# SimeonZhang/detectron2_tensorflow

Measured on AMD Instinct MI355X. Metric: img/sec whole-node Mask R-CNN R50-FPN @1333x800, higher is better.
Workload: dtype f32

## Files before the change

detectron2_tensorflow_amd/csrc/roi_align.hip:

```cpp
#include "common.h"
#include "internal.h"

#include <climits>

namespace d2mi {
namespace {

struct RoiArgs {
  const float* feat[D2MI_MAX_LEVELS];
  float* gfeat[D2MI_MAX_LEVELS];
  int N[D2MI_MAX_LEVELS], H[D2MI_MAX_LEVELS], W[D2MI_MAX_LEVELS];
  float scale[D2MI_MAX_LEVELS];
  int L, C;
  const float* boxes;
  const int32_t* box_ind;
  int R;
  int out_h, out_w, sr, box_mode, pad_border, assign;
  int min_level, max_level, canon_size, canon_level;
  int32_t* level_out;
  float* out;
  const float* gout;
  int32_t* err;
  int bpb;
  int xcd_remap;
// ... 77 lines not shown

__device__ __forceinline__ Tap make_tap(float in, int img_p, int img, bool pad) {
  Tap t;
  t.valid = in >= 0.f && in <= (float)(img_p - 1);
  const float fl = floorf(in);
  const int lo = (int)fl;
  const int hi = (int)ceilf(in);
  t.lerp = in - (float)lo;
  if (pad) {
    t.r0 = min(max(lo - 1, 0), img - 1);
    t.r1 = min(max(hi - 1, 0), img - 1);
  } else {
    t.r0 = min(max(lo, 0), img - 1);
    t.r1 = min(max(hi, 0), img - 1);
  }
  return t;
}

__device__ __forceinline__ float4 lerp4(float4 a, float4 b, float t) {
  return make_float4(a.x + (b.x - a.x) * t, a.y + (b.y - a.y) * t, a.z + (b.z - a.z) * t,
                     a.w + (b.w - a.w) * t);
}

constexpr int kMaxBinsPerBlock = 64, kMinBinsPerBlock = 16, kFwdMinBlocks = 2048;

template <bool VEC4, int U = 4, bool NT = false>
__global__ __launch_bounds__(256) void roi_align_fwd_kernel(RoiArgs a) {
  int r = blockIdx.x;
  if (a.xcd_remap) {
    const int nwg = gridDim.x, q = nwg / 8, r8 = nwg % 8, xcd = r % 8;
    r = (xcd < r8 ? xcd * (q + 1) : r8 * (q + 1) + (xcd - r8) * q) + r / 8;
  }
  const int wave = threadIdx.x >> 6;
  const int lane = threadIdx.x & 63;
  const RoiGeom g = roi_geom(a, r);
  if (threadIdx.x == 0 && blockIdx.y == 0) {
    if (a.level_out) a.level_out[r] = g.lvl;
    if (!g.ok) atomicOr(a.err, kErrBoxInd);
  }
  const int nbins = a.out_h * a.out_w;
  const int S = a.sr > 0 ? a.sr : 1;
  const float inv = a.sr > 0 ? (float)(a.sr * a.sr) : 1.f;
  const float* base = a.feat[g.lvl] + (size_t)(g.ok ? g.n : 0) * g.H * g.W * a.C;
  const int C = a.C;
  const bool pad = a.pad_border != 0;
  const int b_end = min(nbins, (int)(blockIdx.y + 1) * a.bpb);
  if (VEC4 && S == 1 && C == 256) {
    const float4* p = reinterpret_cast<const float4*>(base);
    for (int bb = blockIdx.y * a.bpb + wave; bb < b_end; bb += 4 * U) {
      float4 c00[U], c01[U], c10[U], c11[U];
      float ly[U], lx[U];
      bool ok[U];
#pragma unroll
      for (int u = 0; u < U; ++u) {
        const int bin = min(bb + 4 * u, b_end - 1);
        const int oy = bin / a.out_w, ox = bin - oy * a.out_w;
        const Tap ty = make_tap(in_coord(g.y1, g.y2, g.hs, oy, g.ch, g.Hp), g.Hp, g.H, pad);
        const Tap tx = make_tap(in_coord(g.x1, g.x2, g.ws, ox, g.cw, g.Wp), g.Wp, g.W, pad);
        ok[u] = g.ok && ty.valid && tx.valid;
        ly[u] = ty.lerp;
        lx[u] = tx.lerp;
        c00[u] = p[((size_t)ty.r0 * g.W + tx.r0) * 64 + lane];
        c01[u] = p[((size_t)ty.r0 * g.W + tx.r1) * 64 + lane];
        c10[u] = p[((size_t)ty.r1 * g.W + tx.r0) * 64 + lane];
        c11[u] = p[((size_t)ty.r1 * g.W + tx.r1) * 64 + lane];
      }
#pragma unroll
      for (int u = 0; u < U; ++u) {
        const int bin = bb + 4 * u;
        if (bin >= b_end) break;
        const float4 top = lerp4(c00[u], c01[u], lx[u]);
        const float4 bot = lerp4(c10[u], c11[u], lx[u]);
        const float4 v = ok[u] ? lerp4(top, bot, ly[u]) : make_float4(0.f, 0.f, 0.f, 0.f);
        float4* dst = reinterpret_cast<float4*>(a.out + ((size_t)r * nbins + bin) * C) + lane;
        if (NT) {
          typedef float f4v __attribute__((ext_vector_type(4)));
          __builtin_nontemporal_store(f4v{v.x, v.y, v.z, v.w}, reinterpret_cast<f4v*>(dst));
        } else
          *dst = v;
      }
    }
    return;
  }
  for (int bin = blockIdx.y * a.bpb + wave; bin < b_end; bin += 4) {
    const int oy = bin / a.out_w, ox = bin - oy * a.out_w;
    float* dst = a.out + ((size_t)r * nbins + bin) * C;
    if (VEC4) {
      for (int c4 = lane; c4 * 4 < C; c4 += 64) {
        float4 acc = make_float4(0.f, 0.f, 0.f, 0.f);
        if (g.ok) {
          for (int sy = 0; sy < S; ++sy) {
            const Tap ty = make_tap(in_coord(g.y1, g.y2, g.hs, oy * S + sy, g.ch, g.Hp), g.Hp,
                                    g.H, pad);
            for (int sx = 0; sx < S; ++sx) {
              const Tap tx = make_tap(in_coord(g.x1, g.x2, g.ws, ox * S + sx, g.cw, g.Wp),
                                      g.Wp, g.W, pad);
              float4 v = make_float4(0.f, 0.f, 0.f, 0.f);
              if (ty.valid && tx.valid) {
                const float4* p = reinterpret_cast<const float4*>(base);
                const float4 tl = p[((size_t)ty.r0 * g.W + tx.r0) * (C / 4) + c4];
                const float4 tr = p[((size_t)ty.r0 * g.W + tx.r1) * (C / 4) + c4];
                const float4 bl = p[((size_t)ty.r1 * g.W + tx.r0) * (C / 4) + c4];
                const float4 br = p[((size_t)ty.r1 * g.W + tx.r1) * (C / 4) + c4];
                const float4 top = lerp4(tl, tr, tx.lerp);
                const float4 bot = lerp4(bl, br, tx.lerp);
                v = lerp4(top, bot, ty.lerp);
              }
              if (S == 1) {
                acc = v;
              } else {
                acc.x += v.x; acc.y += v.y; acc.z += v.z; acc.w += v.w;
              }
            }
          }
          if (S > 1) { acc.x /= inv; acc.y /= inv; acc.z /= inv; acc.w /= inv; }
        }
        reinterpret_cast<float4*>(dst)[c4] = acc;
      }
    } else {
      for (int c = lane; c < C; c += 64) {
        float acc = 0.f;
        if (g.ok) {
          for (int sy = 0; sy < S; ++sy) {
            const Tap ty = make_tap(in_coord(g.y1, g.y2, g.hs, oy * S + sy, g.ch, g.Hp), g.Hp,
                                    g.H, pad);
            for (int sx = 0; sx < S; ++sx) {
              const Tap tx = make_tap(in_coord(g.x1, g.x2, g.ws, ox * S + sx, g.cw, g.Wp),
                                      g.Wp, g.W, pad);
              float v = 0.f;
              if (ty.valid && tx.valid) {
                const float tl = base[((size_t)ty.r0 * g.W + tx.r0) * C + c];
                const float tr = base[((size_t)ty.r0 * g.W + tx.r1) * C + c];
                const float bl = base[((size_t)ty.r1 * g.W + tx.r0) * C + c];
                const float br = base[((size_t)ty.r1 * g.W + tx.r1) * C + c];
                const float top = tl + (tr - tl) * tx.lerp;
                const float bot = bl + (br - bl) * tx.lerp;
                v = top + (bot - top) * ty.lerp;
              }
              acc = (S == 1) ? v : acc + v;
            }
          }
          if (S > 1) acc = acc / inv;
        }
        dst[c] = acc;
      }
    }
  }
}

constexpr int kSeg = 64;
constexpr int kBatch = 2;
constexpr int kLongTask = 1024;
constexpr int kLongTile = 4096;

struct PixMap {
  long long base[D2MI_MAX_LEVELS + 1];
  int32_t tbase[D2MI_MAX_LEVELS + 1];
  int L;
};

struct Contrib {
  int32_t row;
  float yl, xl;
  int32_t set;
};

struct RunRec {
  int32_t slot;
  int32_t row;
  float yl, xl;
};

struct BwdCounters {
  int32_t touched, segs, tasks, cursor;
  int32_t touched_lv[D2MI_MAX_LEVELS];
  int32_t touched_hv[D2MI_MAX_LEVELS];
  int32_t lsdone;
};

struct TouchedRange {
  int32_t pre[D2MI_MAX_LEVELS + 1];
  int32_t hv[D2MI_MAX_LEVELS];
  int lo, hi;
  __device__ __forceinline__ void init(const PixMap& pm, const BwdCounters* ctr, int lv_lo,
                                       int lv_hi) {
    lo = lv_lo;
    hi = lv_hi;
    pre[0] = 0;
#pragma unroll
    for (int j = 0; j < D2MI_MAX_LEVELS; ++j) {
      const bool in = j <= hi - lo;
      hv[j] = in ? ctr->touched_hv[lo + j] : 0;
      pre[j + 1] = pre[j] + (in ? ctr->touched_lv[lo + j] + hv[j] : 0);
    }
  }
  __device__ __forceinline__ int total() const {
    int v = 0;
#pragma unroll
    for (int j = 0; j <= D2MI_MAX_LEVELS; ++j) v = j == hi - lo + 1 ? pre[j] : v;
    return v;
  }
  __device__ __forceinline__ long long at(const PixMap& pm, const int32_t* touched, int t,
                                          int& l) const {
    return touched[index(pm, t, l)];
  }
  __device__ __forceinline__ int index(const PixMap& pm, int t, int& l) const {
    int k = 0, base = 0, h = hv[0];
#pragma unroll
    for (int j = 1; j < D2MI_MAX_LEVELS; ++j)
      if (j <= hi - lo && t >= pre[j]) {
        k = j;
        base = pre[j];
        h = hv[j];
      }
    l = lo + k;
    const int kk = t - base;
    return kk < h ? pm.tbase[l + 1] - 1 - kk : pm.tbase[l] + (kk - h);
  }
};

constexpr int kMaxClear = D2MI_MAX_LEVELS + 2;
struct ClearList {
  uint32_t* ptr[kMaxClear];
  long long words[kMaxClear];
  uint32_t value[kMaxClear];
  int n;
};

__global__ __launch_bounds__(256) void roi_bwd_clear_kernel(ClearList cl) {
  const long long tid = (long long)blockIdx.x * blockDim.x + threadIdx.x;
  const long long stride = (long long)gridDim.x * blockDim.x;
  for (int k = 0; k < cl.n; ++k) {
    uint32_t* p = cl.ptr[k];
    const long long n = cl.words[k];
    const uint32_t v = cl.value[k];
    const long long head = std::min<long long>(n, (long long)((16 - ((uintptr_t)p & 15)) & 15) / 4);
    const long long quads = (n - head) / 4;
    uint4* q = reinterpret_cast<uint4*>(p + head);
    const uint4 v4 = make_uint4(v, v, v, v);
    for (long long i = tid; i < quads; i += stride) q[i] = v4;
    const long long tail0 = head + quads * 4;
    if (tid < head) p[tid] = v;
    if (tid < n - tail0) p[tail0 + tid] = v;
  }
}

__device__ __forceinline__ void emit_samples(const RoiArgs& a, const PixMap& pm, int set,
                                             int set_bits, long long sample_base, long long tl,
                                             int32_t* __restrict__ count,
                                             uint64_t* __restrict__ ent,
                                             Contrib* __restrict__ rec) {
  const int S = a.sr > 0 ? a.sr : 1;
  const long long nsamp = (long long)a.out_h * a.out_w * S * S;
  const bool in_range = tl < (long long)a.R * nsamp;
  const int r = in_range ? (int)(tl / nsamp) : 0;
  const int s = in_range ? (int)(tl - (long long)r * nsamp) : 0;
  const RoiGeom g = roi_geom(a, in_range ? r : 0);
  const long long t = sample_base + tl;
  const uint64_t slot = (uint64_t)t * 4u;
  bool ok = in_range && g.ok;
  Tap ty = {}, tx = {};
  int iy = 0, ix = 0;
  if (ok) {
    const bool pad = a.pad_border != 0;
    iy = s / g.cw;
    ix = s - iy * g.cw;
    ty = make_tap(in_coord(g.y1, g.y2, g.hs, iy, g.ch, g.Hp), g.Hp, g.H, pad);
    tx = make_tap(in_coord(g.x1, g.x2, g.ws, ix, g.cw, g.Wp), g.Wp, g.W, pad);
    ok = ty.valid && tx.valid;
  }
  uint32_t q[4] = {0u, 0u, 0u, 0u};
  if (ok) {
    Contrib c;
    c.row = r * (a.out_h * a.out_w) + (iy / S) * a.out_w + ix / S;
    c.yl = ty.lerp;
    c.xl = tx.lerp;
    c.set = set;
    rec[t] = c;
    const uint64_t img = (uint64_t)pm.base[g.lvl] + (uint64_t)g.n * g.H * g.W;
    const uint32_t sb = (uint32_t)set;
    q[0] = (uint32_t)((img + (uint64_t)ty.r0 * g.W + tx.r0) << set_bits) | sb;
    q[1] = (uint32_t)((img + (uint64_t)ty.r0 * g.W + tx.r1) << set_bits) | sb;
    q[2] = (uint32_t)((img + (uint64_t)ty.r1 * g.W + tx.r0) << set_bits) | sb;
    q[3] = (uint32_t)((img + (uint64_t)ty.r1 * g.W + tx.r1) << set_bits) | sb;
  }
  uint32_t rk[4] = {0u, 0u, 0u, 0u};
  const unsigned long long lm = __ballot(ok);
  if (lm != 0) {
    const int lane = threadIdx.x & 63;
    const int lead = __ffsll((long long)lm) - 1;
    bool coll[4];
#pragma unroll
    for (int k = 0; k < 4; ++k) {
      const uint32_t q0 = (uint32_t)__shfl((int)q[k], lead);
      coll[k] = __ballot(ok && q[k] == q0) == lm;
    }
    uint32_t base[4] = {0u, 0u, 0u, 0u};
#pragma unroll
    for (int k = 0; k < 4; ++k) {
      if (coll[k]) {
        if (lane == lead) base[k] = (uint32_t)atomicAdd(&count[q[k]], __popcll(lm));
      } else if (ok) {
        rk[k] = (uint32_t)atomicAdd(&count[q[k]], 1);
      }
    }
#pragma unroll
    for (int k = 0; k < 4; ++k)
      if (coll[k])
        rk[k] = (uint32_t)__shfl((int)base[k], lead) + (uint32_t)__popcll(lm & ((1ull << lane) - 1ull));
  }
  uint64_t e[4];
#pragma unroll
  for (int k = 0; k < 4; ++k) e[k] = ok ? ((uint64_t)q[k] << 32) | rk[k] : ~0ull;
  if (in_range) {
    uint64_t* d = ent + slot;
    d[0] = e[0];
    d[1] = e[1];
    d[2] = e[2];
    d[3] = e[3];
  }
}

__global__ __launch_bounds__(256) void roi_bwd_emit_kernel(RoiArgs a0, RoiArgs a1, int nb0,
                                                           long long ns0, PixMap pm, int set_bits,
                                                           int32_t* __restrict__ count,
                                                           uint64_t* __restrict__ ent,
                                                           Contrib* __restrict__ rec) {
  if ((int)blockIdx.x < nb0)
    emit_samples(a0, pm, 0, set_bits, 0, (long long)blockIdx.x * blockDim.x + threadIdx.x, count,
                 ent, rec);
  else
    emit_samples(a1, pm, 1, set_bits, ns0,
                 (long long)(blockIdx.x - nb0) * blockDim.x + threadIdx.x, count, ent, rec);
}

template <int NT>
__device__ __forceinline__ int wg_alloc(int want, int32_t* __restrict__ counter, int* s_wave,
                                        int* s_base) {
  const int lane = threadIdx.x & 63, w = threadIdx.x >> 6;
  int x = want;
#pragma unroll
  for (int d = 1; d < 64; d <<= 1) {
    const int y = __shfl_up(x, d);
    if (lane >= d) x += y;
  }
  if (lane == 63) s_wave[w] = x;
  __syncthreads();
  if (threadIdx.x == 0) {
    int tot = 0;
    for (int k = 0; k < NT / 64; ++k) {
      const int v = s_wave[k];
      s_wave[k] = tot;
      tot += v;
    }
    *s_base = tot ? atomicAdd(counter, tot) : 0;
  }
  __syncthreads();
  const int off = *s_base + s_wave[w] + x - want;
  __syncthreads();
  return off;
}

template <int NT, int K>
__device__ __forceinline__ void wg_alloc_multi(const int (&want)[K], int32_t* const (&ctr)[K],
                                               int (&off)[K], int (*s_wave)[NT / 64],
                                               int* s_base) {
  const int lane = threadIdx.x & 63, w = threadIdx.x >> 6;
  int x[K];
#pragma unroll
  for (int k = 0; k < K; ++k) x[k] = want[k];
#pragma unroll
  for (int d = 1; d < 64; d <<= 1) {
#pragma unroll
    for (int k = 0; k < K; ++k) {
      const int y = __shfl_up(x[k], d);
      if (lane >= d) x[k] += y;
    }
  }
  if (lane == 63) {
#pragma unroll
    for (int k = 0; k < K; ++k) s_wave[k][w] = x[k];
  }
  __syncthreads();
  if (threadIdx.x < K) {
    const int k = threadIdx.x;
    int tot = 0;
    for (int j = 0; j < NT / 64; ++j) {
      const int v = s_wave[k][j];
      s_wave[k][j] = tot;
      tot += v;
    }
    s_base[k] = tot ? atomicAdd(ctr[k], tot) : 0;
  }
  __syncthreads();
#pragma unroll
  for (int k = 0; k < K; ++k) off[k] = s_base[k] + s_wave[k][w] + x[k] - want[k];
}

__global__ __launch_bounds__(1024) void roi_bwd_runs_kernel(
    const int32_t* __restrict__ count, long long total_pixels, int set_bits,
    int32_t* __restrict__ run_start, int32_t* __restrict__ seg_first,
    int32_t* __restrict__ seg_pixel, int2* __restrict__ tasks, int32_t* __restrict__ touched,
    int4* __restrict__ trun, BwdCounters* __restrict__ ctr, PixMap pm, int heavy_min) {
  __shared__ int s_wave[16], s_base;
  __shared__ int s_wave7[7][16], s_base7[7];
  const long long p = (long long)blockIdx.x * blockDim.x + threadIdx.x;
  const bool live = p < total_pixels;
  const int nsets = 1 << set_bits;
  int c[2] = {0, 0};
  for (int s = 0; s < nsets; ++s) c[s] = live ? count[(p << set_bits) | s] : 0;
  const int tot = c[0] + c[1];
  int nseg[2] = {0, 0}, ntask[2] = {0, 0};
  for (int s = 0; s < nsets; ++s) {
    if (c[s] > kSeg) {
      nseg[s] = (c[s] + kSeg - 1) / kSeg;
      ntask[s] = (c[s] + kLongTask - 1) / kLongTask;
    }
  }
  const long long p0 = (long long)blockIdx.x * blockDim.x;
  const long long p1 = min(p0 + (long long)blockDim.x, total_pixels) - 1;
  int lf = 0, ll = 0, lp = 0;
  while (lf + 1 < pm.L && p0 >= pm.base[lf + 1]) ++lf;
  while (ll + 1 < pm.L && p1 >= pm.base[ll + 1]) ++ll;
  while (lp + 1 < pm.L && p >= pm.base[lp + 1]) ++lp;
  const int l2 = min(lf + 1, ll);
  const bool heavy = heavy_min > 0 && tot > heavy_min, light = tot > 0 && !heavy;
  const int want[7] = {tot, light && lp == lf ? 1 : 0, l2 > lf && light && lp == l2 ? 1 : 0,
                       nseg[0] + nseg[1], ntask[0] + ntask[1], heavy && lp == lf ? 1 : 0,
                       l2 > lf && heavy && lp == l2 ? 1 : 0};
  int32_t* const ctrs[7] = {&ctr->cursor, &ctr->touched_lv[lf], &ctr->touched_lv[l2], &ctr->segs,
                            &ctr->tasks, &ctr->touched_hv[lf], &ctr->touched_hv[l2]};
  int off[7];
  wg_alloc_multi<1024, 7>(want, ctrs, off, s_wave7, s_base7);
  const int pos = off[0], sf = off[3], tf = off[4];
  auto slot_of = [&](int lv, int o_light, int o_heavy) {
    return heavy ? pm.tbase[lv + 1] - 1 - o_heavy : pm.tbase[lv] + o_light;
  };
  int tix = lp == lf ? slot_of(lf, off[1], off[5]) : (lp == l2 ? slot_of(l2, off[2], off[6]) : 0);
  for (int lv = l2 + 1; lv <= ll; ++lv) {
    __syncthreads();
    const int ol = wg_alloc<1024>(light && lp == lv ? 1 : 0, &ctr->touched_lv[lv], s_wave, &s_base);
    const int oh = wg_alloc<1024>(heavy && lp == lv ? 1 : 0, &ctr->touched_hv[lv], s_wave, &s_base);
    if (lp == lv) tix = slot_of(lv, ol, oh);
  }
  if (tot == 0) return;
  touched[tix] = (int32_t)p;
  int o = pos, so = sf, to = tf;
  for (int s = 0; s < nsets; ++s) {
    const int q = (int)((p << set_bits) | s);
    if (trun) trun[((long long)tix << set_bits) | s] = make_int4((int)p, c[s], o, nseg[s] ? so : -1);
    if (c[s] == 0) continue;
    run_start[q] = o;
    o += c[s];
    if (nseg[s]) {
      seg_first[q] = so;
      for (int k = 0; k < nseg[s]; ++k) seg_pixel[so + k] = q;
      so += nseg[s];
      for (int k = 0; k < ntask[s]; ++k) tasks[to + k] = make_int2(q, k);
      to += ntask[s];
    }
  }
}

__global__ __launch_bounds__(256) void roi_bwd_place_kernel(const uint64_t* __restrict__ ent,
                                                            long long n,
                                                            const int32_t* __restrict__ run_start,
                                                            int32_t* __restrict__ arrival,
                                                            const Contrib* __restrict__ rec,
                                                            RunRec* __restrict__ runrec) {
  const long long i = (long long)blockIdx.x * blockDim.x + threadIdx.x;
  if (i >= n) return;
  const uint64_t e = ent[i];
  if (e == ~0ull) return;
  const int q = (int)(e >> 32);
  const int pos = run_start[q] + (int)(uint32_t)e;
  arrival[pos] = (int32_t)i;
  if (runrec) {
    const Contrib c = rec[i >> 2];
    runrec[pos] = RunRec{(int32_t)i, c.row, c.yl, c.xl};
  }
}

struct BinDiv {
  float inv, rcp;
  bool pow2;
};
__device__ __forceinline__ BinDiv bin_div(int sr) {
  const int n = sr * sr;
  return BinDiv{(float)n, 1.f / (float)n, n > 0 && (n & (n - 1)) == 0};
}
__device__ __forceinline__ float4 div4(float4 g, const BinDiv& d) {
  if (d.pow2) return make_float4(g.x * d.rcp, g.y * d.rcp, g.z * d.rcp, g.w * d.rcp);
  return make_float4(g.x / d.inv, g.y / d.inv, g.z / d.inv, g.w / d.inv);
}

__device__ __forceinline__ float weigh(int corner, float yl, float xl, float v) {
  const float d = (corner < 2) ? (1.f - yl) * v : yl * v;
  return (corner & 1) ? xl * d : (1.f - xl) * d;
}

template <bool VEC4>
__device__ __forceinline__ float4 sum_slots(const RoiArgs& a, const int32_t* slots,
                                            const Contrib* __restrict__ rec, int n, int c,
                                            bool live) {
  float4 acc = make_float4(0.f, 0.f, 0.f, 0.f);
  const int C = a.C;
  for (int i = 0; i < n; i += kBatch) {
    int corner[kBatch];
    Contrib e[kBatch];
    const int m = min(kBatch, n - i);
#pragma unroll
    for (int u = 0; u < kBatch; ++u) {
      if (u < m) {
        const int slot = slots[i + u];
        corner[u] = slot & 3;
        e[u] = rec[slot >> 2];
      }
    }
    float4 v[kBatch] = {};
#pragma unroll
    for (int u = 0; u < kBatch; ++u) {
      if (u < m && live) {
        const float* src = a.gout_s[e[u].set] + (size_t)e[u].row * C + c;
        if (VEC4) v[u] = *reinterpret_cast<const float4*>(src);
        else v[u].x = *src;
      }
    }
#pragma unroll
    for (int u = 0; u < kBatch; ++u) {
      if (u < m) {
        float4 g = v[u];
        const int sr = a.sr_s[e[u].set];
        if (sr > 0) g = div4(g, bin_div(sr));
        acc.x += weigh(corner[u], e[u].yl, e[u].xl, g.x);
        if (VEC4) {
          acc.y += weigh(corner[u], e[u].yl, e[u].xl, g.y);
          acc.z += weigh(corner[u], e[u].yl, e[u].xl, g.z);
          acc.w += weigh(corner[u], e[u].yl, e[u].xl, g.w);
        }
      }
    }
  }
  return acc;
}

template <int G>
__device__ __forceinline__ void order_run(const int32_t* __restrict__ arrival, int i0, int n,
                                          int sub, int32_t* in, int32_t* out) {
  constexpr int K = kSeg / G;
  int v[K];
#pragma unroll
  for (int k = 0; k < K; ++k) {
    const int idx = sub + k * G;
    v[k] = idx < n ? arrival[i0 + idx] : INT_MAX;
    if (idx < n) in[idx] = v[k];
  }
  __builtin_amdgcn_wave_barrier();
  int rank[K] = {};
  for (int j = 0; j < n; ++j) {
    const int o = in[j];
#pragma unroll
    for (int k = 0; k < K; ++k) rank[k] += o < v[k] ? 1 : 0;
  }
#pragma unroll
  for (int k = 0; k < K; ++k)
    if (sub + k * G < n) out[rank[k]] = v[k];
  __builtin_amdgcn_wave_barrier();
}

template <bool VEC4>
__global__ __launch_bounds__(1024) void roi_bwd_long_kernel(
    RoiArgs a, const int32_t* __restrict__ arrival, const int32_t* __restrict__ count,
    const int32_t* __restrict__ run_start, const int2* __restrict__ tasks,
    BwdCounters* __restrict__ ctr, int32_t* __restrict__ sorted_long,
    const Contrib* __restrict__ rec, const int32_t* __restrict__ seg_first,
    const int32_t* __restrict__ seg_pixel, float* __restrict__ partial) {
  __shared__ int32_t tile[kLongTile];
  __shared__ int s_last;
  const int ntasks = ctr->tasks;
  for (int tk = blockIdx.x; tk < ntasks; tk += gridDim.x) {
    const int2 task = tasks[tk];
    const int i0 = run_start[task.x], len = count[task.x];
    const int e = task.y * kLongTask + (int)threadIdx.x;
    const int mine = e < len ? arrival[i0 + e] : INT_MAX;
    int rank = 0;
    for (int j0 = 0; j0 < len; j0 += kLongTile) {
      const int m = min(kLongTile, len - j0);
      __syncthreads();
      for (int j = threadIdx.x; j < m; j += blockDim.x) tile[j] = arrival[i0 + j0 + j];
      __syncthreads();
      int j = 0;
      for (; j + 8 <= m; j += 8) {
#pragma unroll
        for (int u = 0; u < 8; ++u) rank += tile[j + u] < mine ? 1 : 0;
      }
      for (; j < m; ++j) rank += tile[j] < mine ? 1 : 0;
    }
    if (e < len) sorted_long[i0 + rank] = mine;
    __syncthreads();
  }
  __syncthreads();
  if (threadIdx.x == 0) {
    __threadfence();
    s_last = atomicAdd(&ctr->lsdone, 1) == (int)gridDim.x - 1;
  }
  __syncthreads();
  if (!s_last) return;
  __threadfence();
  const int lane = threadIdx.x & 63, nw = blockDim.x >> 6;
  const int nsegs = ctr->segs;
  const int step = VEC4 ? 256 : 64;
  for (int seg = threadIdx.x >> 6; seg < nsegs; seg += nw) {
    const int q = seg_pixel[seg];
    const int k = seg - seg_first[q];
    const int i0 = run_start[q] + k * kSeg;
    const int n = min(kSeg, count[q] - k * kSeg);
    for (int c0 = 0; c0 < a.C; c0 += step) {
      const int c = c0 + (VEC4 ? lane * 4 : lane);
      const bool live = c < a.C;
      const float4 acc = sum_slots<VEC4>(a, sorted_long + i0, rec, n, c, live);
      if (live) {
        float* dst = partial + (size_t)seg * a.C + c;
        if (VEC4) *reinterpret_cast<float4*>(dst) = acc;
        else *dst = acc.x;
      }
    }
  }
}

template <bool VEC4>
__global__ __launch_bounds__(256) void roi_bwd_pixel_kernel(
    RoiArgs a, PixMap pm, const int32_t* __restrict__ arrival, const Contrib* __restrict__ rec,
    int set_bits, const int32_t* __restrict__ count, const int32_t* __restrict__ run_start,
    const int32_t* __restrict__ seg_first, const float* __restrict__ partial,
    const int32_t* __restrict__ touched, const BwdCounters* __restrict__ ctr, int lv_lo,
    int lv_hi) {
  __shared__ int32_t lds[4][2][kSeg];
  const int lane = threadIdx.x & 63, w = threadIdx.x >> 6;
  const int C = a.C;
  const int step = VEC4 ? 256 : 64;
  TouchedRange tr;
  tr.init(pm, ctr, lv_lo, lv_hi);
  const int nt = tr.total();
  const int nsets = 1 << set_bits;
  for (int t = blockIdx.x * 4 + w; t < nt; t += gridDim.x * 4) {
    int l;
    const long long pix = tr.at(pm, touched, t, l);
    float* dst = a.gfeat[l] + (size_t)(pix - pm.base[l]) * C;
    const bool acc_lv = (a.acc_mask >> l) & 1;
    for (int c0 = 0; c0 < C; c0 += step) {
      const int c = c0 + (VEC4 ? lane * 4 : lane);
      const bool live = c < C;
      float4 res = make_float4(0.f, 0.f, 0.f, 0.f);
      bool any = false;
      for (int sidx = 0; sidx < nsets; ++sidx) {
        const long long q = (pix << set_bits) | sidx;
        const int n = count[q];
        if (n == 0) continue;
        const int i0 = run_start[q];
        float4 acc = make_float4(0.f, 0.f, 0.f, 0.f);
        if (n <= kSeg) {
          order_run<64>(arrival, i0, n, lane, lds[w][0], lds[w][1]);
          acc = sum_slots<VEC4>(a, lds[w][1], rec, n, c, live);
        } else if (live) {
          const int f = seg_first[q];
          const int ns = (n + kSeg - 1) / kSeg;
          for (int j = 0; j < ns; ++j) {
            const float* src = partial + (size_t)(f + j) * C + c;
            if (VEC4) {
              const float4 v = *reinterpret_cast<const float4*>(src);
              acc.x += v.x; acc.y += v.y; acc.z += v.z; acc.w += v.w;
            } else {
              acc.x += *src;
            }
          }
        }
        if (any) {
          res.x = res.x + acc.x; res.y = res.y + acc.y; res.z = res.z + acc.z; res.w = res.w + acc.w;
        } else {
          res = acc;
          any = true;
        }
      }
      if (live) {
        if (VEC4) {
          if (acc_lv) {
            const float4 o = *reinterpret_cast<const float4*>(dst + c);
            res.x = o.x + res.x;
            res.y = o.y + res.y;
            res.z = o.z + res.z;
            res.w = o.w + res.w;
          }
          *reinterpret_cast<float4*>(dst + c) = res;
        } else {
          dst[c] = acc_lv ? dst[c] + res.x : res.x;
        }
      }
    }
  }
}

__global__ __launch_bounds__(256) void roi_bwd_pixel_c256_kernel(
    RoiArgs a, PixMap pm, const RunRec* __restrict__ runrec, int set_bits,
    const int4* __restrict__ trun, const float* __restrict__ partial,
    const BwdCounters* __restrict__ ctr, int lv_lo, int lv_hi) {
  constexpr int C = 256;
  constexpr int PPW = 2, kRowBatch = 4;
  constexpr int LPP = 64 / PPW;
  constexpr int F = C / LPP / 4;
  constexpr int KR = kSeg / LPP;
  __shared__ int32_t lslot[4][PPW][kSeg];
  __shared__ int4 lrec[4][PPW][kSeg];
  const int lane = threadIdx.x & 63, w = threadIdx.x >> 6;
  const int grp = lane / LPP, sub = lane % LPP;
  const int c = sub * 4 * F;
  TouchedRange tr;
  tr.init(pm, ctr, lv_lo, lv_hi);
  const int nt = tr.total();
  const int nsets = 1 << set_bits;
  int32_t* lin = lslot[w][grp];
  int4* lout = lrec[w][grp];
  const int wave = blockIdx.x * 4 + w;
  for (int tb = wave * PPW; tb < nt; tb += gridDim.x * 4 * PPW) {
    const int t = tb + grp;
    if (t >= nt) continue;
    int l;
    const int ti = tr.index(pm, t, l);
    const int4 ru0 = trun[(long long)ti << set_bits];
    const int4 ru1 = set_bits ? trun[((long long)ti << set_bits) | 1] : make_int4(0, 0, 0, -1);
    const long long pix = ru0.x;
    float* dst = a.gfeat[l] + (size_t)(pix - pm.base[l]) * C + c;
    float4* d4 = reinterpret_cast<float4*>(dst);
    const bool acc_lv = (a.acc_mask >> l) & 1;
    float4 old[F];
    if (acc_lv) {
#pragma unroll
      for (int k = 0; k < F; ++k) old[k] = d4[k];
    }
    float4 res[F];
    bool any = false;
    for (int sidx = 0; sidx < nsets; ++sidx) {
      const int4 ru = sidx ? ru1 : ru0;
      const int n = ru.y;
      if (n == 0) continue;
      const int i0 = ru.z;
      float4 acc[F];
#pragma unroll
      for (int k = 0; k < F; ++k) acc[k] = make_float4(0.f, 0.f, 0.f, 0.f);
      if (n <= kSeg) {
        int4 v[KR];
#pragma unroll
        for (int k = 0; k < KR; ++k) {
          const int idx = sub + k * LPP;
          v[k] = idx < n ? *reinterpret_cast<const int4*>(runrec + i0 + idx)
                         : make_int4(INT_MAX, 0, 0, 0);
          if (idx < n) lin[idx] = v[k].x;
        }
        __builtin_amdgcn_wave_barrier();
        int rank[KR] = {};
        for (int j = 0; j < n; ++j) {
          const int o = lin[j];
#pragma unroll
          for (int k = 0; k < KR; ++k) rank[k] += o < v[k].x ? 1 : 0;
        }
#pragma unroll
// ... 10 lines not shown
          for (int u = 0; u < kRowBatch; ++u) {
            if (i + u < n) {
              e[u] = lout[i + u];
              const float4* src = reinterpret_cast<const float4*>(gout + (size_t)e[u].y * C + c);
#pragma unroll
              for (int k = 0; k < F; ++k) vv[u][k] = src[k];
            }
          }
#pragma unroll
          for (int u = 0; u < kRowBatch; ++u) {
            if (i + u < n) {
              const int corner = e[u].x & 3;
              const float yl = __int_as_float(e[u].z), xl = __int_as_float(e[u].w);
#pragma unroll
              for (int k = 0; k < F; ++k) {
                float4 g = vv[u][k];
                if (sr > 0) g = div4(g, bd);
                acc[k].x += weigh(corner, yl, xl, g.x);
                acc[k].y += weigh(corner, yl, xl, g.y);
                acc[k].z += weigh(corner, yl, xl, g.z);
                acc[k].w += weigh(corner, yl, xl, g.w);
              }
            }
          }
        }
        __builtin_amdgcn_wave_barrier();
      } else {
        const int f = ru.w;
        const int ns = (n + kSeg - 1) / kSeg;
        for (int j = 0; j < ns; ++j) {
          const float4* src = reinterpret_cast<const float4*>(partial + (size_t)(f + j) * C + c);
#pragma unroll
          for (int k = 0; k < F; ++k) {
            const float4 v = src[k];
            acc[k].x += v.x; acc[k].y += v.y; acc[k].z += v.z; acc[k].w += v.w;
          }
        }
      }
#pragma unroll
      for (int k = 0; k < F; ++k) {
        if (any) {
          res[k].x = res[k].x + acc[k].x; res[k].y = res[k].y + acc[k].y;
          res[k].z = res[k].z + acc[k].z; res[k].w = res[k].w + acc[k].w;
        } else {
          res[k] = acc[k];
        }
      }
      any = true;
    }
    if (!any) continue;
#pragma unroll
    for (int k = 0; k < F; ++k) {
      if (acc_lv) {
        const float4 o = old[k];
        res[k].x = o.x + res[k].x; res[k].y = o.y + res[k].y;
        res[k].z = o.z + res[k].z; res[k].w = o.w + res[k].w;
      }
      d4[k] = res[k];
    }
  }
}

int fill_args(RoiArgs& a, const int32_t* dims, const float* scales, int num_levels, int C,
              const float* boxes, const int32_t* box_ind, int R, int out_h, int out_w,
              int sampling_ratio, int box_mode, int pad_border, int assign, int min_level,
              int max_level, int canonical_box_size, int canonical_level) {
  D2MI_REQUIRE(num_levels >= 1 && num_levels <= D2MI_MAX_LEVELS, "num_levels=%d out of [1,%d]",
               num_levels, D2MI_MAX_LEVELS);
  D2MI_REQUIRE(C > 0 && R >= 0 && out_h > 0 && out_w > 0, "bad ROIAlign sizes C=%d R=%d out=%dx%d",
               C, R, out_h, out_w);
  D2MI_REQUIRE(sampling_ratio >= 0, "sampling_ratio must be >= 0, got %d", sampling_ratio);
  D2MI_REQUIRE(box_mode >= 0 && box_mode <= 2, "box_mode must be 0, 1 or 2");
  D2MI_REQUIRE(!(assign && num_levels > 1) || (max_level - min_level + 1 == num_levels),
               "level range %d..%d does not match num_levels=%d", min_level, max_level,
               num_levels);
  D2MI_REQUIRE(canonical_box_size > 0, "canonical_box_size must be > 0");
  D2MI_REQUIRE(((uintptr_t)boxes & 15) == 0, "boxes must be 16-byte aligned");
  a.L = num_levels;
  a.C = C;
  for (int l = 0; l < num_levels; ++l) {
    a.N[l] = dims[3 * l];
    a.H[l] = dims[3 * l + 1];
    a.W[l] = dims[3 * l + 2];
    a.scale[l] = scales[l];
    D2MI_REQUIRE(a.H[l] > 0 && a.W[l] > 0, "level %d has empty spatial size", l);
  }
  a.boxes = boxes;
  a.box_ind = box_ind;
  a.R = R;
  a.out_h = out_h;
  a.out_w = out_w;
  a.sr = sampling_ratio;
  a.box_mode = box_mode;
  a.pad_border = pad_border;
  a.assign = assign;
  a.min_level = min_level;
  a.max_level = max_level;
  a.canon_size = canonical_box_size;
  a.canon_level = canonical_level;
  a.err = error_word();
  D2MI_REQUIRE(a.err != nullptr, "device error word unavailable");
  return 0;
}

}
}

using namespace d2mi;

extern "C" int d2mi_roi_align_fwd(const float* const* feats, const int32_t* dims,
                                  const float* scales, int num_levels, int C, const float* boxes,
                                  const int32_t* box_ind, int R, int out_h, int out_w,
                                  int sampling_ratio, int box_mode, int pad_border, int assign,
                                  int min_level, int max_level, int canonical_box_size,
                                  int canonical_level, int32_t* level_out, float* out,
                                  void* stream) {
  RoiArgs a = {};
  int rc = fill_args(a, dims, scales, num_levels, C, boxes, box_ind, R, out_h, out_w,
                     sampling_ratio, box_mode, pad_border, assign, min_level, max_level,
                     canonical_box_size, canonical_level);
  if (rc) return rc;
  bool vec4 = (C % 4) == 0 && ((uintptr_t)out & 15) == 0;
  for (int l = 0; l < num_levels; ++l) {
    a.feat[l] = feats[l];
    vec4 = vec4 && (((uintptr_t)feats[l] & 15) == 0);
  }
  a.level_out = level_out;
  a.out = out;
  if (R == 0) return 0;
  const int nbins = out_h * out_w;
  a.bpb = kMaxBinsPerBlock;
  while (a.bpb > kMinBinsPerBlock &&
         (long long)R * ((nbins + a.bpb - 1) / a.bpb) < kFwdMinBlocks)
    a.bpb /= 2;
  const int nby = (nbins + a.bpb - 1) / a.bpb;
  a.bpb = (nbins + nby - 1) / nby;
  a.xcd_remap = 1;
  dim3 grid(R, nby);
  hipStream_t st = as_stream(stream);
  if (!vec4)
    hipLaunchKernelGGL((roi_align_fwd_kernel<false>), grid, dim3(256), 0, st, a);
  else if (R >= 256)
    hipLaunchKernelGGL((roi_align_fwd_kernel<true, 2, true>), grid, dim3(256), 0, st, a);
  else
    hipLaunchKernelGGL((roi_align_fwd_kernel<true, 4, true>), grid, dim3(256), 0, st, a);
  D2MI_LAUNCH_CHECK();
  return 0;
}

namespace d2mi {
namespace {

struct BwdPlan {
  long long total_pixels, pairs, n_keys, n_samples, max_segs, max_touched, max_tasks;
  int set_bits;
  PixMap pm;
};

int bwd_plan_n(const int32_t* dims, int num_levels, long long n_samples, int set_bits,
               BwdPlan* p) {
  p->n_samples = n_samples;
  p->n_keys = p->n_samples * 4;
  p->set_bits = set_bits;
  long long t = 0;
  for (int l = 0; l < num_levels; ++l) {
    p->pm.base[l] = t;
    t += (long long)dims[3 * l] * dims[3 * l + 1] * dims[3 * l + 2];
  }
  p->pm.base[num_levels] = t;
  p->pm.L = num_levels;
  p->total_pixels = t;
  p->pairs = t << set_bits;
  p->max_segs = 2 * (p->n_keys / kSeg) + 1;
  p->max_tasks = p->n_keys / kLongTask + p->n_keys / (kSeg + 1) + 2;
  p->pm.tbase[0] = 0;
  for (int l = 0; l < num_levels; ++l)
    p->pm.tbase[l + 1] =
        p->pm.tbase[l] + (int32_t)std::min(p->n_keys, p->pm.base[l + 1] - p->pm.base[l]);
  p->max_touched = p->pm.tbase[num_levels];
  D2MI_REQUIRE(p->n_keys < (1LL << 31) && p->pairs < (1LL << 31) &&
                   p->n_keys * num_levels < (1LL << 31),
               "ROIAlign backward too large");
  return 0;
}

int bwd_plan(const int32_t* dims, int num_levels, int R, int out_h, int out_w, int sr,
             BwdPlan* p) {
  const long long S = sr > 0 ? sr : 1;
  return bwd_plan_n(dims, num_levels, (long long)R * out_h * out_w * S * S, 0, p);
}

struct BwdSpace {
  uint64_t* ent;
  int32_t* arrival;
  RunRec* runrec;
  int32_t* sorted_long;
  Contrib* rec;
  int32_t *count, *run_start, *seg_first, *seg_pixel;
  float* partial;
  int32_t* touched;
  int4* trun;
  int2* tasks;
  BwdCounters* ctr;
  template <typename A>
  void lay(A& w, int C, const BwdPlan& p) {
    ent = w.template take<uint64_t>((size_t)p.n_keys + 1);
    arrival = w.template take<int32_t>((size_t)p.n_keys + 1);
    runrec = w.template take<RunRec>((size_t)p.n_keys + 1);
    sorted_long = w.template take<int32_t>((size_t)p.n_keys + 1);
    rec = w.template take<Contrib>((size_t)p.n_samples + 1);
    count = w.template take<int32_t>((size_t)p.pairs + 1);
    run_start = w.template take<int32_t>((size_t)p.pairs + 1);
    seg_first = w.template take<int32_t>((size_t)p.pairs + 1);
    seg_pixel = w.template take<int32_t>((size_t)p.max_segs);
    partial = w.template take<float>((size_t)p.max_segs * C);
    touched = w.template take<int32_t>((size_t)p.max_touched + 1);
    trun = w.template take<int4>(((size_t)p.max_touched + 1) * 2);
    tasks = w.template take<int2>((size_t)p.max_tasks);
    ctr = w.template take<BwdCounters>(1);
  }
};

int roi_bwd_core(const RoiArgs* sets, int nsets, const int32_t* dims, int num_levels, int C,
                 int acc_mask, bool vec4, void* workspace, size_t workspace_bytes,
                 hipStream_t st, int phase = 3, int lv_lo = 0, int lv_hi = -1) {
  if (lv_hi < 0) lv_hi = num_levels - 1;
  D2MI_REQUIRE(phase >= 1 && phase <= 3 && 0 <= lv_lo && lv_lo <= lv_hi && lv_hi < num_levels,
               "ROIAlign backward: bad phase %d / level range [%d, %d]", phase, lv_lo, lv_hi);
  RoiArgs a = sets[0];
  a.acc_mask = acc_mask;
  long long ns[2] = {0, 0};
  for (int k = 0; k < nsets; ++k) {
    const long long S = sets[k].sr > 0 ? sets[k].sr : 1;
    ns[k] = (long long)sets[k].R * sets[k].out_h * sets[k].out_w * S * S;
    a.gout_s[k] = sets[k].gout;
    a.sr_s[k] = sets[k].sr;
  }
  const int sb = nsets > 1 ? 1 : 0;
  BwdPlan p;
  int rc = bwd_plan_n(dims, num_levels, ns[0] + ns[1], sb, &p);
  if (rc) return rc;
  Workspace w(workspace, workspace_bytes);
  BwdSpace s;
  s.lay(w, C, p);
  D2MI_REQUIRE(w.ok() && (workspace || w.off == 0),
               "ROIAlign backward workspace too small: %zu < %zu", workspace_bytes, w.off);
  if (p.total_pixels == 0) return 0;
  const bool use_runrec = vec4 && C == 256;
  if (phase & 1) {
  ClearList cl = {};
  long long clear_words = 0;
  auto clear = [&](void* ptr, long long words, uint32_t value) {
    cl.ptr[cl.n] = static_cast<uint32_t*>(ptr);
    cl.words[cl.n] = words;
    cl.value[cl.n] = value;
    ++cl.n;
    clear_words += words;
  };
  for (int l = lv_lo; l <= lv_hi; ++l)
    if (!((acc_mask >> l) & 1))
      clear(a.gfeat[l], (long long)dims[3 * l] * dims[3 * l + 1] * dims[3 * l + 2] * C, 0u);
  clear(s.count, p.pairs, 0u);
  clear(s.ctr, sizeof(BwdCounters) / 4, 0u);
  hipLaunchKernelGGL(roi_bwd_clear_kernel,
                     dim3((unsigned)std::max(1LL, std::min((clear_words / 4 + 255) / 256, 8192LL))),
                     dim3(256), 0, st, cl);
  D2MI_LAUNCH_CHECK();
  if (p.n_keys == 0) return 0;
  {
    const int nb0 = (int)((ns[0] + 255) / 256), nb1 = nsets > 1 ? (int)((ns[1] + 255) / 256) : 0;
    if (nb0 + nb1 > 0) {
      hipLaunchKernelGGL(roi_bwd_emit_kernel, dim3((unsigned)(nb0 + nb1)), dim3(256), 0, st,
                         sets[0], sets[nsets > 1 ? 1 : 0], nb0, ns[0], p.pm, sb, s.count, s.ent,
                         s.rec);
      D2MI_LAUNCH_CHECK();
    }
  }
  hipLaunchKernelGGL(roi_bwd_runs_kernel, dim3((unsigned)((p.total_pixels + 1023) / 1024)),
                     dim3(1024), 0, st, s.count, p.total_pixels, sb, s.run_start, s.seg_first,
                     s.seg_pixel, s.tasks, s.touched, use_runrec ? s.trun : nullptr, s.ctr, p.pm,
                     tuning(kTuneRoiHeavy));
  D2MI_LAUNCH_CHECK();
  hipLaunchKernelGGL(roi_bwd_place_kernel, dim3((unsigned)((p.n_keys + 255) / 256)), dim3(256), 0,
                     st, s.ent, p.n_keys, s.run_start, s.arrival, s.rec,
                     use_runrec ? s.runrec : nullptr);
  D2MI_LAUNCH_CHECK();
  hipLaunchKernelGGL((vec4 ? roi_bwd_long_kernel<true> : roi_bwd_long_kernel<false>),
                     dim3((unsigned)std::max(1LL, std::min<long long>(p.max_tasks, 64LL))),
                     dim3(1024), 0, st, a, s.arrival, s.count, s.run_start, s.tasks, s.ctr,
                     s.sorted_long, s.rec, s.seg_first, s.seg_pixel, s.partial);
  D2MI_LAUNCH_CHECK();
  }
  if (phase == 2) {
    ClearList cl = {};
    long long words = 0;
    for (int l = lv_lo; l <= lv_hi; ++l)
      if (!((acc_mask >> l) & 1)) {
        cl.ptr[cl.n] = reinterpret_cast<uint32_t*>(a.gfeat[l]);
        cl.words[cl.n] = (long long)dims[3 * l] * dims[3 * l + 1] * dims[3 * l + 2] * C;
        words += cl.words[cl.n++];
      }
    if (cl.n) {
      hipLaunchKernelGGL(roi_bwd_clear_kernel,
                         dim3((unsigned)std::max(1LL, std::min((words / 4 + 255) / 256, 8192LL))),
                         dim3(256), 0, st, cl);
      D2MI_LAUNCH_CHECK();
    }
  }
  if (!(phase & 2) || p.n_keys == 0) return 0;
  const long long cap = p.pm.tbase[lv_hi + 1] - p.pm.tbase[lv_lo];
  const long long wg_max = std::max(1, tuning(kTuneRoiPixGrid));
  const dim3 grid((unsigned)std::max(1LL, std::min((cap + 3) / 4, wg_max)));
  if (use_runrec) {
    const dim3 g4((unsigned)std::max(1LL, std::min((cap + 7) / 8, wg_max)));
    hipLaunchKernelGGL(roi_bwd_pixel_c256_kernel, g4, dim3(256), 0, st, a, p.pm, s.runrec, sb,
                       s.trun, s.partial, s.ctr, lv_lo, lv_hi);
  } else if (vec4) {
    hipLaunchKernelGGL(roi_bwd_pixel_kernel<true>, grid, dim3(256), 0, st, a, p.pm, s.arrival,
                       s.rec, sb, s.count, s.run_start, s.seg_first, s.partial, s.touched, s.ctr,
                       lv_lo, lv_hi);
  } else {
    hipLaunchKernelGGL(roi_bwd_pixel_kernel<false>, grid, dim3(256), 0, st, a, p.pm, s.arrival,
                       s.rec, sb, s.count, s.run_start, s.seg_first, s.partial, s.touched, s.ctr,
                       lv_lo, lv_hi);
  }
  D2MI_LAUNCH_CHECK();
  return 0;
}

}
}

extern "C" size_t d2mi_roi_align_bwd_workspace_size(const int32_t* dims, int num_levels, int C,
                                                    int R, int out_h, int out_w,
                                                    int sampling_ratio) {
  if (!dims || num_levels < 1 || num_levels > D2MI_MAX_LEVELS || R < 0 || C < 1) return 0;
  BwdPlan p;
  if (bwd_plan(dims, num_levels, R, out_h, out_w, sampling_ratio, &p)) return 0;
  return layout_bytes<BwdSpace>(C, p);
}

extern "C" int d2mi_roi_align_bwd_ex(float* const* grad_feats, const int32_t* dims,
                                     const float* scales, int num_levels, int C,
                                     const float* boxes, const int32_t* box_ind, int R, int out_h,
                                     int out_w, int sampling_ratio, int box_mode, int pad_border,
                                     int assign, int min_level, int max_level,
                                     int canonical_box_size, int canonical_level,
                                     const float* grad_out, int accumulate, void* workspace,
                                     size_t workspace_bytes, void* stream) {
  RoiArgs a = {};
  int rc = fill_args(a, dims, scales, num_levels, C, boxes, box_ind, R, out_h, out_w,
                     sampling_ratio, box_mode, pad_border, assign, min_level, max_level,
                     canonical_box_size, canonical_level);
  if (rc) return rc;
  bool vec4 = (C % 4) == 0 && ((uintptr_t)grad_out & 15) == 0;
  for (int l = 0; l < num_levels; ++l) {
    a.gfeat[l] = grad_feats[l];
    vec4 = vec4 && (((uintptr_t)grad_feats[l] & 15) == 0);
  }
  a.gout = grad_out;
  return roi_bwd_core(&a, 1, dims, num_levels, C, accumulate ? (1 << num_levels) - 1 : 0, vec4,
                      workspace, workspace_bytes, as_stream(stream));
}

extern "C" size_t d2mi_roi_align_bwd2_workspace_size(const int32_t* dims, int num_levels, int C,
                                                     int R0, int out_h0, int out_w0, int sr0,
                                                     int R1, int out_h1, int out_w1, int sr1) {
  if (!dims || num_levels < 1 || num_levels > D2MI_MAX_LEVELS || R0 < 0 || R1 < 0 || C < 1)
    return 0;
  const long long S0 = sr0 > 0 ? sr0 : 1, S1 = sr1 > 0 ? sr1 : 1;
  BwdPlan p;
  if (bwd_plan_n(dims, num_levels,
                 (long long)R0 * out_h0 * out_w0 * S0 * S0 + (long long)R1 * out_h1 * out_w1 * S1 * S1,
                 1, &p))
    return 0;
  return layout_bytes<BwdSpace>(C, p);
}

extern "C" int d2mi_roi_align_bwd2_ex(float* const* grad_feats, const int32_t* dims,
                                      const float* scales, int num_levels, int C, int box_mode,
                                      int pad_border, int assign, int min_level, int max_level,
                                      int canonical_box_size, int canonical_level,
                                      const float* boxes0, const int32_t* box_ind0, int R0,
                                      int out_h0, int out_w0, int sr0, const float* grad_out0,
                                      const float* boxes1, const int32_t* box_ind1, int R1,
                                      int out_h1, int out_w1, int sr1, const float* grad_out1,
                                      int accumulate_mask, int phase, int level_lo, int level_hi,
                                      void* workspace, size_t workspace_bytes, void* stream) {
  RoiArgs sets[2] = {};
  int rc = fill_args(sets[0], dims, scales, num_levels, C, boxes0, box_ind0, R0, out_h0, out_w0,
                     sr0, box_mode, pad_border, assign, min_level, max_level, canonical_box_size,
                     canonical_level);
  if (rc) return rc;
  rc = fill_args(sets[1], dims, scales, num_levels, C, boxes1, box_ind1, R1, out_h1, out_w1, sr1,
                 box_mode, pad_border, assign, min_level, max_level, canonical_box_size,
                 canonical_level);
  if (rc) return rc;
  bool vec4 = (C % 4) == 0 && ((uintptr_t)grad_out0 & 15) == 0 && ((uintptr_t)grad_out1 & 15) == 0;
  for (int l = 0; l < num_levels; ++l) {
    sets[0].gfeat[l] = sets[1].gfeat[l] = grad_feats ? grad_feats[l] : nullptr;
    vec4 = vec4 && (((uintptr_t)sets[0].gfeat[l] & 15) == 0);
  }
  sets[0].gout = grad_out0;
  sets[1].gout = grad_out1;
  D2MI_REQUIRE((accumulate_mask >> num_levels) == 0, "accumulate_mask has bits past the levels");
  for (int l = level_lo; l <= level_hi && l < num_levels; ++l)
    D2MI_REQUIRE(l < 0 || sets[0].gfeat[l] != nullptr ||
                     (phase == 1 && ((accumulate_mask >> l) & 1)),
                 "level %d's gradient map is needed by this phase", l);
  return roi_bwd_core(sets, 2, dims, num_levels, C, accumulate_mask, vec4, workspace,
                      workspace_bytes, as_stream(stream), phase, level_lo, level_hi);
}

extern "C" int d2mi_roi_align_bwd2(float* const* grad_feats, const int32_t* dims,
                                   const float* scales, int num_levels, int C, int box_mode,
                                   int pad_border, int assign, int min_level, int max_level,
                                   int canonical_box_size, int canonical_level,
                                   const float* boxes0, const int32_t* box_ind0, int R0,
                                   int out_h0, int out_w0, int sr0, const float* grad_out0,
                                   const float* boxes1, const int32_t* box_ind1, int R1,
                                   int out_h1, int out_w1, int sr1, const float* grad_out1,
                                   int accumulate_mask, void* workspace, size_t workspace_bytes,
                                   void* stream) {
  return d2mi_roi_align_bwd2_ex(grad_feats, dims, scales, num_levels, C, box_mode, pad_border,
                                assign, min_level, max_level, canonical_box_size, canonical_level,
                                boxes0, box_ind0, R0, out_h0, out_w0, sr0, grad_out0, boxes1,
                                box_ind1, R1, out_h1, out_w1, sr1, grad_out1, accumulate_mask, 3, 0,
                                num_levels - 1, workspace, workspace_bytes, stream);
}

extern "C" int d2mi_roi_align_bwd(float* const* grad_feats, const int32_t* dims,
                                  const float* scales, int num_levels, int C, const float* boxes,
                                  const int32_t* box_ind, int R, int out_h, int out_w,
                                  int sampling_ratio, int box_mode, int pad_border, int assign,
                                  int min_level, int max_level, int canonical_box_size,
                                  int canonical_level, const float* grad_out, void* workspace,
                                  size_t workspace_bytes, void* stream) {
  return d2mi_roi_align_bwd_ex(grad_feats, dims, scales, num_levels, C, boxes, box_ind, R, out_h,
                               out_w, sampling_ratio, box_mode, pad_border, assign, min_level,
                               max_level, canonical_box_size, canonical_level, grad_out, 0,
                               workspace, workspace_bytes, stream);
}
```

Baseline: 111.9.

## Split ROIAlign backward long-run kernel into rank and partial kernels

The single long-run kernel, which ranked arrivals and then had one last block compute every segment partial, becomes two kernels. The rank kernel runs with 256-thread blocks, has each thread rank four elements per task, and sends runs of at most 1024 entries to per-wave order_run sorts through a new wtasks list. The partial kernel spreads segment partials over a grid of up to 512 blocks, replacing the serial last-block tail. The cost is one extra launch, an extra workspace buffer and a changed task sizing, which adds risk if the new bounds are wrong.

```diff
diff --git a/detectron2_tensorflow_amd/csrc/roi_align.hip b/detectron2_tensorflow_amd/csrc/roi_align.hip
--- a/detectron2_tensorflow_amd/csrc/roi_align.hip
+++ b/detectron2_tensorflow_amd/csrc/roi_align.hip
@@ -253,6 +253,7 @@
 constexpr int kBatch = 2;
 constexpr int kLongTask = 1024;
 constexpr int kLongTile = 4096;
+constexpr int kRankGrid = 256, kPartialGrid = 512;
 
 struct PixMap {
   long long base[D2MI_MAX_LEVELS + 1];
@@ -276,7 +277,7 @@
   int32_t touched, segs, tasks, cursor;
   int32_t touched_lv[D2MI_MAX_LEVELS];
   int32_t touched_hv[D2MI_MAX_LEVELS];
-  int32_t lsdone;
+  int32_t wtasks;
 };
 
 struct TouchedRange {
@@ -501,21 +502,23 @@
 __global__ __launch_bounds__(1024) void roi_bwd_runs_kernel(
     const int32_t* __restrict__ count, long long total_pixels, int set_bits,
     int32_t* __restrict__ run_start, int32_t* __restrict__ seg_first,
-    int32_t* __restrict__ seg_pixel, int2* __restrict__ tasks, int32_t* __restrict__ touched,
-    int4* __restrict__ trun, BwdCounters* __restrict__ ctr, PixMap pm, int heavy_min) {
+    int32_t* __restrict__ seg_pixel, int2* __restrict__ tasks, int32_t* __restrict__ wtasks,
+    int32_t* __restrict__ touched, int4* __restrict__ trun, BwdCounters* __restrict__ ctr,
+    PixMap pm, int heavy_min) {
   __shared__ int s_wave[16], s_base;
-  __shared__ int s_wave7[7][16], s_base7[7];
+  __shared__ int s_wave8[8][16], s_base8[8];
   const long long p = (long long)blockIdx.x * blockDim.x + threadIdx.x;
   const bool live = p < total_pixels;
   const int nsets = 1 << set_bits;
   int c[2] = {0, 0};
   for (int s = 0; s < nsets; ++s) c[s] = live ? count[(p << set_bits) | s] : 0;
   const int tot = c[0] + c[1];
-  int nseg[2] = {0, 0}, ntask[2] = {0, 0};
+  int nseg[2] = {0, 0}, ntask[2] = {0, 0}, nwtask[2] = {0, 0};
   for (int s = 0; s < nsets; ++s) {
     if (c[s] > kSeg) {
       nseg[s] = (c[s] + kSeg - 1) / kSeg;
-      ntask[s] = (c[s] + kLongTask - 1) / kLongTask;
+      if (c[s] <= kLongTask) nwtask[s] = 1;
+      else ntask[s] = (c[s] + kLongTask - 1) / kLongTask;
     }
   }
   const long long p0 = (long long)blockIdx.x * blockDim.x;
@@ -526,14 +529,15 @@
   while (lp + 1 < pm.L && p >= pm.base[lp + 1]) ++lp;
   const int l2 = min(lf + 1, ll);
   const bool heavy = heavy_min > 0 && tot > heavy_min, light = tot > 0 && !heavy;
-  const int want[7] = {tot, light && lp == lf ? 1 : 0, l2 > lf && light && lp == l2 ? 1 : 0,
+  const int want[8] = {tot, light && lp == lf ? 1 : 0, l2 > lf && light && lp == l2 ? 1 : 0,
                        nseg[0] + nseg[1], ntask[0] + ntask[1], heavy && lp == lf ? 1 : 0,
-                       l2 > lf && heavy && lp == l2 ? 1 : 0};
-  int32_t* const ctrs[7] = {&ctr->cursor, &ctr->touched_lv[lf], &ctr->touched_lv[l2], &ctr->segs,
-                            &ctr->tasks, &ctr->touched_hv[lf], &ctr->touched_hv[l2]};
-  int off[7];
-  wg_alloc_multi<1024, 7>(want, ctrs, off, s_wave7, s_base7);
-  const int pos = off[0], sf = off[3], tf = off[4];
+                       l2 > lf && heavy && lp == l2 ? 1 : 0, nwtask[0] + nwtask[1]};
+  int32_t* const ctrs[8] = {&ctr->cursor, &ctr->touched_lv[lf], &ctr->touched_lv[l2], &ctr->segs,
+                            &ctr->tasks, &ctr->touched_hv[lf], &ctr->touched_hv[l2],
+                            &ctr->wtasks};
+  int off[8];
+  wg_alloc_multi<1024, 8>(want, ctrs, off, s_wave8, s_base8);
+  const int pos = off[0], sf = off[3], tf = off[4], wf = off[7];
   auto slot_of = [&](int lv, int o_light, int o_heavy) {
     return heavy ? pm.tbase[lv + 1] - 1 - o_heavy : pm.tbase[lv] + o_light;
   };
@@ -546,7 +550,7 @@
   }
   if (tot == 0) return;
   touched[tix] = (int32_t)p;
-  int o = pos, so = sf, to = tf;
+  int o = pos, so = sf, to = tf, wo = wf;
   for (int s = 0; s < nsets; ++s) {
     const int q = (int)((p << set_bits) | s);
     if (trun) trun[((long long)tix << set_bits) | s] = make_int4((int)p, c[s], o, nseg[s] ? so : -1);
@@ -559,6 +563,7 @@
       so += nseg[s];
       for (int k = 0; k < ntask[s]; ++k) tasks[to + k] = make_int2(q, k);
       to += ntask[s];
+      if (nwtask[s]) wtasks[wo++] = q;
     }
   }
 }
@@ -645,10 +650,9 @@
   return acc;
 }
 
-template <int G>
+template <int G, int K = kSeg / G>
 __device__ __forceinline__ void order_run(const int32_t* __restrict__ arrival, int i0, int n,
                                           int sub, int32_t* in, int32_t* out) {
-  constexpr int K = kSeg / G;
   int v[K];
 #pragma unroll
   for (int k = 0; k < K; ++k) {
@@ -669,49 +673,72 @@
   __builtin_amdgcn_wave_barrier();
 }
 
-template <bool VEC4>
-__global__ __launch_bounds__(1024) void roi_bwd_long_kernel(
-    RoiArgs a, const int32_t* __restrict__ arrival, const int32_t* __restrict__ count,
+__global__ __launch_bounds__(256) void roi_bwd_rank_kernel(
+    const int32_t* __restrict__ arrival, const int32_t* __restrict__ count,
     const int32_t* __restrict__ run_start, const int2* __restrict__ tasks,
-    BwdCounters* __restrict__ ctr, int32_t* __restrict__ sorted_long,
-    const Contrib* __restrict__ rec, const int32_t* __restrict__ seg_first,
-    const int32_t* __restrict__ seg_pixel, float* __restrict__ partial) {
+    const int32_t* __restrict__ wtasks, const BwdCounters* __restrict__ ctr,
+    int32_t* __restrict__ sorted_long) {
+  constexpr int NT = 256, EPT = kLongTask / NT;
+  static_assert(kLongTile == (NT / 64) * kLongTask, "a wave's run is its quarter of the tile");
   __shared__ int32_t tile[kLongTile];
-  __shared__ int s_last;
-  const int ntasks = ctr->tasks;
+  const int ntasks = ctr->tasks, nwtasks = ctr->wtasks;
   for (int tk = blockIdx.x; tk < ntasks; tk += gridDim.x) {
     const int2 task = tasks[tk];
     const int i0 = run_start[task.x], len = count[task.x];
-    const int e = task.y * kLongTask + (int)threadIdx.x;
-    const int mine = e < len ? arrival[i0 + e] : INT_MAX;
-    int rank = 0;
+    int mine[EPT], rank[EPT];
+#pragma unroll
+    for (int k = 0; k < EPT; ++k) {
+      const int e = task.y * kLongTask + k * NT + (int)threadIdx.x;
+      mine[k] = e < len ? arrival[i0 + e] : INT_MAX;
+      rank[k] = 0;
+    }
     for (int j0 = 0; j0 < len; j0 += kLongTile) {
       const int m = min(kLongTile, len - j0);
       __syncthreads();
-      for (int j = threadIdx.x; j < m; j += blockDim.x) tile[j] = arrival[i0 + j0 + j];
+      for (int j = threadIdx.x; j < m; j += NT) tile[j] = arrival[i0 + j0 + j];
       __syncthreads();
       int j = 0;
-      for (; j + 8 <= m; j += 8) {
-#pragma unroll
-        for (int u = 0; u < 8; ++u) rank += tile[j + u] < mine ? 1 : 0;
-      }
-      for (; j < m; ++j) rank += tile[j] < mine ? 1 : 0;
-    }
-    if (e < len) sorted_long[i0 + rank] = mine;
-    __syncthreads();
+      for (; j + 4 <= m; j += 4) {
+#pragma unroll
+        for (int u = 0; u < 4; ++u) {
+          const int o = tile[j + u];
+#pragma unroll
+          for (int k = 0; k < EPT; ++k) rank[k] += o < mine[k] ? 1 : 0;
+        }
+      }
+      for (; j < m; ++j) {
+        const int o = tile[j];
+#pragma unroll
+        for (int k = 0; k < EPT; ++k) rank[k] += o < mine[k] ? 1 : 0;
+      }
+    }
+#pragma unroll
+    for (int k = 0; k < EPT; ++k)
+      if (task.y * kLongTask + k * NT + (int)threadIdx.x < len) sorted_long[i0 + rank[k]] = mine[k];
   }
   __syncthreads();
-  if (threadIdx.x == 0) {
-    __threadfence();
-    s_last = atomicAdd(&ctr->lsdone, 1) == (int)gridDim.x - 1;
-  }
-  __syncthreads();
-  if (!s_last) return;
-  __threadfence();
-  const int lane = threadIdx.x & 63, nw = blockDim.x >> 6;
+  const int lane = threadIdx.x & 63, w = threadIdx.x >> 6;
+  int32_t* row = tile + w * kLongTask;
+  for (int tk = blockIdx.x * (NT / 64) + w; tk < nwtasks; tk += gridDim.x * (NT / 64)) {
+    const int q = wtasks[tk];
+    const int i0 = run_start[q], n = min(count[q], kLongTask);
+    if (n <= 128) order_run<64, 2>(arrival, i0, n, lane, row, sorted_long + i0);
+    else if (n <= 256) order_run<64, 4>(arrival, i0, n, lane, row, sorted_long + i0);
+    else if (n <= 512) order_run<64, 8>(arrival, i0, n, lane, row, sorted_long + i0);
+    else order_run<64, 16>(arrival, i0, n, lane, row, sorted_long + i0);
+  }
+}
+
+template <bool VEC4>
+__global__ __launch_bounds__(256) void roi_bwd_partial_kernel(
+    RoiArgs a, const int32_t* __restrict__ count, const int32_t* __restrict__ run_start,
+    const BwdCounters* __restrict__ ctr, const int32_t* __restrict__ sorted_long,
+    const Contrib* __restrict__ rec, const int32_t* __restrict__ seg_first,
+    const int32_t* __restrict__ seg_pixel, float* __restrict__ partial) {
+  const int lane = threadIdx.x & 63, nw = gridDim.x * (blockDim.x >> 6);
   const int nsegs = ctr->segs;
   const int step = VEC4 ? 256 : 64;
-  for (int seg = threadIdx.x >> 6; seg < nsegs; seg += nw) {
+  for (int seg = blockIdx.x * (blockDim.x >> 6) + (threadIdx.x >> 6); seg < nsegs; seg += nw) {
     const int q = seg_pixel[seg];
     const int k = seg - seg_first[q];
     const int i0 = run_start[q] + k * kSeg;
@@ -1028,7 +1055,7 @@
 namespace {
 
 struct BwdPlan {
-  long long total_pixels, pairs, n_keys, n_samples, max_segs, max_touched, max_tasks;
+  long long total_pixels, pairs, n_keys, n_samples, max_segs, max_touched, max_tasks, max_wtasks;
   int set_bits;
   PixMap pm;
 };
@@ -1048,7 +1075,8 @@
   p->total_pixels = t;
   p->pairs = t << set_bits;
   p->max_segs = 2 * (p->n_keys / kSeg) + 1;
-  p->max_tasks = p->n_keys / kLongTask + p->n_keys / (kSeg + 1) + 2;
+  p->max_wtasks = p->n_keys / (kSeg + 1) + 1;
+  p->max_tasks = 2 * (p->n_keys / kLongTask) + 2;
   p->pm.tbase[0] = 0;
   for (int l = 0; l < num_levels; ++l)
     p->pm.tbase[l + 1] =
@@ -1077,6 +1105,7 @@
   int32_t* touched;
   int4* trun;
   int2* tasks;
+  int32_t* wtasks;
   BwdCounters* ctr;
   template <typename A>
   void lay(A& w, int C, const BwdPlan& p) {
@@ -1093,6 +1122,7 @@
     touched = w.template take<int32_t>((size_t)p.max_touched + 1);
     trun = w.template take<int4>(((size_t)p.max_touched + 1) * 2);
     tasks = w.template take<int2>((size_t)p.max_tasks);
+    wtasks = w.template take<int32_t>((size_t)p.max_wtasks);
     ctr = w.template take<BwdCounters>(1);
   }
 };
@@ -1154,17 +1184,24 @@
   }
   hipLaunchKernelGGL(roi_bwd_runs_kernel, dim3((unsigned)((p.total_pixels + 1023) / 1024)),
                      dim3(1024), 0, st, s.count, p.total_pixels, sb, s.run_start, s.seg_first,
-                     s.seg_pixel, s.tasks, s.touched, use_runrec ? s.trun : nullptr, s.ctr, p.pm,
-                     tuning(kTuneRoiHeavy));
+                     s.seg_pixel, s.tasks, s.wtasks, s.touched, use_runrec ? s.trun : nullptr,
+                     s.ctr, p.pm, tuning(kTuneRoiHeavy));
   D2MI_LAUNCH_CHECK();
   hipLaunchKernelGGL(roi_bwd_place_kernel, dim3((unsigned)((p.n_keys + 255) / 256)), dim3(256), 0,
                      st, s.ent, p.n_keys, s.run_start, s.arrival, s.rec,
                      use_runrec ? s.runrec : nullptr);
   D2MI_LAUNCH_CHECK();
-  hipLaunchKernelGGL((vec4 ? roi_bwd_long_kernel<true> : roi_bwd_long_kernel<false>),
-                     dim3((unsigned)std::max(1LL, std::min<long long>(p.max_tasks, 64LL))),
-                     dim3(1024), 0, st, a, s.arrival, s.count, s.run_start, s.tasks, s.ctr,
-                     s.sorted_long, s.rec, s.seg_first, s.seg_pixel, s.partial);
+  hipLaunchKernelGGL(roi_bwd_rank_kernel,
+                     dim3((unsigned)std::max(
+                         1LL, std::min<long long>(p.max_tasks + (p.max_wtasks + 3) / 4, kRankGrid))),
+                     dim3(256), 0, st, s.arrival, s.count, s.run_start, s.tasks, s.wtasks, s.ctr,
+                     s.sorted_long);
+  D2MI_LAUNCH_CHECK();
+  hipLaunchKernelGGL((vec4 ? roi_bwd_partial_kernel<true> : roi_bwd_partial_kernel<false>),
+                     dim3((unsigned)std::max(
+                         1LL, std::min<long long>((p.max_segs + 3) / 4, kPartialGrid))),
+                     dim3(256), 0, st, a, s.count, s.run_start, s.ctr, s.sorted_long, s.rec,
+                     s.seg_first, s.seg_pixel, s.partial);
   D2MI_LAUNCH_CHECK();
   }
   if (phase == 2) {
```

Result: no change. 113.0 (median of 6 runs) (+1.0%).
